# CCIG-Champalimaud/adell-mri

Measured on AMD Instinct MI355X. Metric: volumes/sec 3D U-Net 128^3 2-ch seg (train step: fwd+loss+bwd+SGD), higher is better.
Workload: dtype f32 (f16x3 split MFMA, fp32 accumulate); 1 GPU; BASELINE configs[1]: u-net-3d-resnet.yaml UNetPL, 2x128^3, batch 2/GPU, dice+focal, SGD-Nesterov; per_gpu_batch=2, parallelism=dp1, yaml=configs/u-net-3d-resnet.yaml, built_by=parse_config_unet -> get_segmentation_network('unet'), gradient_exchange=none (1 rank)

## Files before the change

adell_mri_amd/csrc/conv_fwd_s2.hip:

```cpp
#include <type_traits>
#include <utility>
#include "common.h"

typedef _Float16 half8 __attribute__((ext_vector_type(8)));
typedef _Float16 half4 __attribute__((ext_vector_type(4)));

namespace {

constexpr int kHX = 9, kHY = 9, kHZ = 5, kHV = kHX * kHY * kHZ;
constexpr int kWBytes = 27 * 2 * 32 * 64;
constexpr int kImg = kHV * 64;
constexpr int kCW = 4, kPW = 4;
constexpr int kThreads = (kCW + kPW) * 64, kPThreads = kPW * 64;
constexpr int kRedFloats = kCW * 32 * 2;
constexpr int kLds = kWBytes + 2 * kImg + 64 + kRedFloats * 4;
static_assert(kLds <= 160 * 1024, "one block per CU: weights + two half images");
constexpr int kItems = kHV * 4;
constexpr int kPer = (kItems + kPThreads - 1) / kPThreads;

template <typename T>
__device__ __forceinline__ ADELL_GLOBAL T* uniform_ptr(T* p) {
  const uint64_t v = reinterpret_cast<uint64_t>(p);
  const uint32_t lo = __builtin_amdgcn_readfirstlane((uint32_t)v);
  const uint32_t hi = __builtin_amdgcn_readfirstlane((uint32_t)(v >> 32));
  return reinterpret_cast<ADELL_GLOBAL T*>(((uint64_t)hi << 32) | lo);
}

template <int N, typename F, int... I>
__device__ __forceinline__ void static_for_impl(F&& body, std::integer_sequence<int, I...>) {
  (body(std::integral_constant<int, I>{}), ...);
}
template <int N, typename F>
__device__ __forceinline__ void static_for(F&& body) {
  static_for_impl<N>(body, std::make_integer_sequence<int, N>{});
}

struct FwdS2Args {
  const float* x;
  const char* wpack;
  const float* wscale;
  const float* bias;
  float* y;
  float* part;
  unsigned* amax_out;
  int N, D, H, W, Do, Ho, Wo;
  int ntx, nty, ntz;
  int nbricks;
};

}

#define ADELL_S2_BARRIER() asm volatile("s_waitcnt lgkmcnt(0)\n\ts_barrier" ::: "memory")

__device__ __forceinline__ int fwd_s2_scale_exp(float mx) {
  int kA = 0;
  const int ebits = (__float_as_int(mx) >> 23) & 0xff;
  if (ebits > 0 && ebits < 255) kA = 8 * ((13 - (ebits - 127)) >> 3);
  if (kA > 96) kA = 96;
  if (kA < -96) kA = -96;
  return kA;
}

__device__ __forceinline__ float fwd_s2_wave_max(float v) {
  auto step = [&](auto CTRL, auto ROWS) {
    const int o = __builtin_amdgcn_update_dpp(__float_as_int(v), __float_as_int(v), decltype(CTRL)::value,
                                              decltype(ROWS)::value, 0xf, false);
    v = fmaxf(v, __int_as_float(o));
  };
  step(std::integral_constant<int, 0xB1>{}, std::integral_constant<int, 0xf>{});
  step(std::integral_constant<int, 0x4E>{}, std::integral_constant<int, 0xf>{});
  step(std::integral_constant<int, 0x141>{}, std::integral_constant<int, 0xf>{});
  step(std::integral_constant<int, 0x140>{}, std::integral_constant<int, 0xf>{});
  step(std::integral_constant<int, 0x142>{}, std::integral_constant<int, 0xa>{});
  step(std::integral_constant<int, 0x143>{}, std::integral_constant<int, 0xc>{});
  return __int_as_float(__builtin_amdgcn_readlane(__float_as_int(v), 63));
}

template <int DBG>
__global__ __launch_bounds__(kThreads, 1) void adell_fwd_s2_fused_kernel(FwdS2Args a) {
  extern __shared__ char smem[];
  char* sW = smem;
  char* sA = smem + kWBytes;
  float* sMax = reinterpret_cast<float*>(sA + 2 * kImg);
  float* sRed = sMax + 16;
  const int tid = threadIdx.x, lane = tid & 63, wave = tid >> 6;
  const int li = lane & 31, lh = lane >> 5;
  const int nsp = a.ntx * a.nty * a.ntz;

  int first, stride, count;
  if (gridDim.x >= 8) {
    const int xcd = blockIdx.x & 7, per = (a.nbricks + 7) >> 3;
    const int lo = xcd * per, hi = (lo + per < a.nbricks) ? lo + per : a.nbricks;
    stride = gridDim.x >> 3;
    first = lo + (blockIdx.x >> 3);
    count = first < hi ? (hi - 1 - first) / stride + 1 : 0;
  } else {
    stride = gridDim.x;
    first = blockIdx.x;
    count = first < a.nbricks ? (a.nbricks - 1 - first) / stride + 1 : 0;
  }
  if (count == 0) return;
  const int nphases = count * 8;

  auto brick_origin = [&](int t, int& nb, int& tile, int& ox0, int& oy0, int& oz0) {
    tile = t % nsp;
    nb = t / nsp;
    int r = tile;
    const int tx = r % a.ntx;
    r /= a.ntx;
    const int ty = r % a.nty;
    const int tz = r / a.nty;
    ox0 = tx * 8;
    oy0 = ty * 8;
    oz0 = tz * 4;
  };

#pragma unroll 7
  for (int it = tid; it < 27 * 256; it += kThreads) {
    const float4 v = *reinterpret_cast<const float4*>(a.wpack + (size_t)it * 16);
    const int slot = it & 3, row = it >> 2;
    const int ch = row & 1, n = (row >> 1) & 31, tap = row >> 6;
    *reinterpret_cast<float4*>(sW + ((tap * 2 + ch) * 32 + n) * 64 + ((slot ^ ((n >> 2) & 3)) << 4)) = v;
  }

  if (wave >= kCW) {
    const int ptid = tid - kCW * 64, pw = wave - kCW;
    unsigned reloff[kPer], ldsoff[kPer];
#pragma unroll
    for (int u = 0; u < kPer; ++u) {
      int j = ptid + kPThreads * u;
      j = j < kItems ? j : j - kItems;
      const int hv = j >> 2, q4 = j & 3;
      const int hz = hv / (kHX * kHY), rem = hv - hz * (kHX * kHY);
      const int hy = rem / kHX, hx = rem - hy * kHX;
      reloff[u] = (unsigned)((2 * hz * a.H + 2 * hy) * a.W + 2 * hx) * 32u + 4u * q4;
      const int sw = (hv >> 2) & 3;
      ldsoff[u] = (unsigned)(hv * 64 + (q4 & 1) * 8 + (((q4 >> 1) ^ sw) << 4)) |
                  (unsigned)((hx << 16) | (hy << 20) | (hz << 24));
    }
    float4 raw[2][2][kPer];
    unsigned okbuf[2] = {0u, 0u};
    int pf_nb = 0, pf_ox0 = 0, pf_oy0 = 0, pf_oz0 = 0;
    auto issue = [&](int p, float4 (&f)[2][kPer], unsigned& okbits) {
      const int cls = p & 7;
      if (cls == 0) {
        int tile;
        brick_origin(first + (p >> 3) * stride, pf_nb, tile, pf_ox0, pf_oy0, pf_oz0);
        pf_nb = __builtin_amdgcn_readfirstlane(pf_nb);
        pf_ox0 = __builtin_amdgcn_readfirstlane(pf_ox0);
        pf_oy0 = __builtin_amdgcn_readfirstlane(pf_oy0);
        pf_oz0 = __builtin_amdgcn_readfirstlane(pf_oz0);
      }
      const int pz = cls >> 2, py = (cls >> 1) & 1, px = cls & 1;
      const int bz = 2 * (pf_oz0 - 1) + pz, by = 2 * (pf_oy0 - 1) + py, bx = 2 * (pf_ox0 - 1) + px;
      const ADELL_GLOBAL float* src = uniform_ptr(a.x + (size_t)pf_nb * a.D * a.H * a.W * 32);
      const bool inside = (bz >= 0) & (by >= 0) & (bx >= 0) & (bz + 2 * (kHZ - 1) < a.D) &
                          (by + 2 * (kHY - 1) < a.H) & (bx + 2 * (kHX - 1) < a.W);
      unsigned rel[kPer];
      unsigned ok = 0;
      if (inside) {
        const unsigned base = (unsigned)((bz * a.H + by) * a.W + bx) * 32u;
#pragma unroll
        for (int u = 0; u < kPer; ++u) rel[u] = base + reloff[u];
        ok = 0x80000000u;
      } else {
        const int base = ((bz * a.H + by) * a.W + bx) * 32;
#pragma unroll
        for (int u = 0; u < kPer; ++u) {
          const int hx = (ldsoff[u] >> 16) & 15, hy = (ldsoff[u] >> 20) & 15, hz = ldsoff[u] >> 24;
          const int iz = bz + 2 * hz, iy = by + 2 * hy, ix = bx + 2 * hx;
          const bool v = (iz >= 0) & (iz < a.D) & (iy >= 0) & (iy < a.H) & (ix >= 0) & (ix < a.W);
          rel[u] = v ? (unsigned)(base + (int)reloff[u]) : 0u;
          ok |= v ? (1u << u) : 0u;
        }
      }
      okbits = ok;
#pragma unroll
      for (int u = 0; u < kPer; ++u) {
        const f32x4 v0 = *reinterpret_cast<const ADELL_GLOBAL f32x4*>(src + rel[u]);
        const f32x4 v1 = *reinterpret_cast<const ADELL_GLOBAL f32x4*>(src + rel[u] + 16);
        f[0][u] = make_float4(v0.x, v0.y, v0.z, v0.w);
        f[1][u] = make_float4(v1.x, v1.y, v1.z, v1.w);
      }
    };
    auto publish_max = [&](float4 (&f)[2][kPer], unsigned okbits, int row) {
      float mx = 0.f;
#pragma unroll
      for (int c = 0; c < 2; ++c) {
        if (!(okbits >> 31)) {
#pragma unroll
          for (int u = 0; u < kPer; ++u) {
            const bool ok = (okbits >> u) & 1u;
            f[c][u] = make_float4(ok ? f[c][u].x : 0.f, ok ? f[c][u].y : 0.f, ok ? f[c][u].z : 0.f,
                                  ok ? f[c][u].w : 0.f);
          }
        }
#pragma unroll
        for (int u = 0; u < kPer; ++u)
          mx = fmaxf(fmaxf(fmaxf(mx, fabsf(f[c][u].x)), fmaxf(fabsf(f[c][u].y), fabsf(f[c][u].z))),
                     fabsf(f[c][u].w));
      }
      mx = fwd_s2_wave_max(mx);
      if (lane == 0) sMax[row * kPW + pw] = mx;
    };
    auto convert = [&](const float4 (&f)[kPer], float scaleA, char* img) {
#pragma unroll
      for (int u = 0; u < kPer; ++u) {
        if (!(DBG & 8)) {
          const float v[4] = {f[u].x * scaleA, f[u].y * scaleA, f[u].z * scaleA, f[u].w * scaleA};
          half4 h, l;
#pragma unroll
          for (int j = 0; j < 4; ++j) {
            h[j] = (_Float16)v[j];
            l[j] = (_Float16)(v[j] - (float)h[j]);
          }
          const unsigned off = ldsoff[u] & 0xffffu;
          *reinterpret_cast<half4*>(img + off) = h;
          *reinterpret_cast<half4*>(img + (off ^ 32u)) = l;
        }
      }
    };

    float block_max = 0.f;
    issue(0, raw[0], okbuf[0]);
    issue(1, raw[1], okbuf[1]);
    publish_max(raw[0], okbuf[0], 0);
    ADELL_S2_BARRIER();
    auto pstep = [&](int p, auto BUF) __attribute__((always_inline)) {
      constexpr int B = decltype(BUF)::value;
      const float* sm = sMax + kPW * (p & 1);
      const float mx = fmaxf(fmaxf(sm[0], sm[1]), fmaxf(sm[2], sm[3]));
      block_max = fmaxf(block_max, mx);
      const float scaleA = __int_as_float((fwd_s2_scale_exp(mx) + 127) << 23);
      const int pn = p + 2 < nphases ? p + 2 : nphases - 1;
      convert(raw[B][0], scaleA, sA);
      ADELL_S2_BARRIER();
      convert(raw[B][1], scaleA, sA + kImg);
      if (!((DBG & 16) && p > 1)) issue(pn, raw[B], okbuf[B]);
      publish_max(raw[1 - B], okbuf[1 - B], (p + 1) & 1);
      ADELL_S2_BARRIER();
    };
    for (int p = 0; p < nphases; p += 2) {
      pstep(p, std::integral_constant<int, 0>{});
      pstep(p + 1, std::integral_constant<int, 1>{});
    }
    ADELL_S2_BARRIER();
    if (a.amax_out != nullptr && ptid == 0) atomicMax(a.amax_out, __float_as_uint(block_max));
    return;
  }

  const int wz = wave;
  int arow[2];
#pragma unroll
  for (int mt = 0; mt < 2; ++mt) arow[mt] = (wz * kHY + (li >> 3) + 4 * mt) * kHX + (li & 7);
  const int bsw = (li >> 2) & 3;
  const int boffh = li * 64 + ((lh ^ bsw) << 4), boffl = li * 64 + (((2 + lh) ^ bsw) << 4);
  const float wsc = a.wscale[li];
  const float bcol = a.bias ? a.bias[li] : 0.f;
  f32x16 acc[2];
  int kprev = 0;

  auto taps = [&](int cls, auto CHT) __attribute__((always_inline)) {
    constexpr int ch = decltype(CHT)::value;
    const char* sAc = sA + ch * kImg;
    static_for<8>([&](auto CLS) {
      constexpr int c = decltype(CLS)::value;
      if (cls == c) {
        constexpr int pz = c >> 2, py = (c >> 1) & 1, px = c & 1;
        static_for<8>([&](auto T) {
          constexpr int tb = decltype(T)::value;
          constexpr int sz = tb >> 2, sy = (tb >> 1) & 1, sx = tb & 1;
          if constexpr ((sz <= pz) && (sy <= py) && (sx <= px) && !(DBG & 1)) {
            constexpr int tz = pz ? 2 * sz : 1, ty = py ? 2 * sy : 1, tx = px ? 2 * sx : 1;
            constexpr int dz = pz ? sz : 1, dy = py ? sy : 1, dx = px ? sx : 1;
            constexpr int tap = (tz * 3 + ty) * 3 + tx;
            const char* bt = sW + (tap * 2 + ch) * (32 * 64);
            const half8 bh = *reinterpret_cast<const half8*>(bt + boffh);
            const half8 bl = *reinterpret_cast<const half8*>(bt + boffl);
#pragma unroll
            for (int mt = 0; mt < 2; ++mt) {
              const int hv = arow[mt] + (dz * kHY + dy) * kHX + dx;
              const int sw = (hv >> 2) & 3;
              const char* row = sAc + hv * 64;
              const half8 ah = *reinterpret_cast<const half8*>(row + ((lh ^ sw) << 4));
              const half8 al = *reinterpret_cast<const half8*>(row + (((2 + lh) ^ sw) << 4));
              acc[mt] = __builtin_amdgcn_mfma_f32_32x32x16_f16(al, bh, acc[mt], 0, 0, 0);
              acc[mt] = __builtin_amdgcn_mfma_f32_32x32x16_f16(ah, bl, acc[mt], 0, 0, 0);
              acc[mt] = __builtin_amdgcn_mfma_f32_32x32x16_f16(ah, bh, acc[mt], 0, 0, 0);
            }
          }
        });
      }
    });
  };
  auto fold_stats = [&](int i) {
    if (a.part && tid < 32 && !(DBG & 2)) {
      int nb, tile, ox0, oy0, oz0;
      brick_origin(first + i * stride, nb, tile, ox0, oy0, oz0);
      float t1 = 0.f, t2 = 0.f;
#pragma unroll
      for (int w = 0; w < kCW; ++w) {
        t1 += sRed[(w * 32 + tid) * 2 + 0];
        t2 += sRed[(w * 32 + tid) * 2 + 1];
      }
      float* p = a.part + (((size_t)nb * nsp + tile) * 32 + tid) * 2;
      p[0] = t1;
      p[1] = t2;
    }
  };

  ADELL_S2_BARRIER();
  for (int p = 0; p < nphases; ++p) {
    const int cls = p & 7;
    {
      const float* sm = sMax + kPW * (p & 1);
      const float mx = fmaxf(fmaxf(sm[0], sm[1]), fmaxf(sm[2], sm[3]));
      const int kA = fwd_s2_scale_exp(mx);
      if (cls == 0) {
#pragma unroll
        for (int mt = 0; mt < 2; ++mt)
#pragma unroll
          for (int r = 0; r < 16; ++r) acc[mt][r] = 0.f;
      } else if (kA != kprev) {
        const float fix = __int_as_float((kA - kprev + 127) << 23);
#pragma unroll
        for (int mt = 0; mt < 2; ++mt)
#pragma unroll
          for (int r = 0; r < 16; ++r) acc[mt][r] *= fix;
      }
      kprev = kA;
    }
    ADELL_S2_BARRIER();
    if (cls == 0 && p > 0) fold_stats((p >> 3) - 1);
    taps(cls, std::integral_constant<int, 0>{});
    ADELL_S2_BARRIER();
    taps(cls, std::integral_constant<int, 1>{});
    if (cls == 7) {
      int nb, tile, ox0, oy0, oz0;
      brick_origin(first + (p >> 3) * stride, nb, tile, ox0, oy0, oz0);
      const float oscale = __int_as_float((127 - kprev) << 23) * wsc;
      const int z = oz0 + wz;
      float s1 = 0.f, s2 = 0.f;
      if (z < a.Do && !(DBG & 2)) {
#pragma unroll
        for (int mt = 0; mt < 2; ++mt)
#pragma unroll
          for (int r = 0; r < 16; ++r) {
            const int x = ox0 + (r & 3) + 4 * lh, yy = oy0 + (r >> 2) + 4 * mt;
            if (x < a.Wo && yy < a.Ho) {
              const float v = acc[mt][r] * oscale + bcol;
              a.y[((((size_t)nb * a.Do + z) * a.Ho + yy) * a.Wo + x) * 32 + li] = v;
              s1 += v;
              s2 += v * v;
            }
          }
      }
      if (a.part) {
        s1 += __shfl_xor(s1, 32, 64);
        s2 += __shfl_xor(s2, 32, 64);
        if (lh == 0) {
          sRed[(wz * 32 + li) * 2 + 0] = s1;
          sRed[(wz * 32 + li) * 2 + 1] = s2;
        }
      }
    }
  }
  ADELL_S2_BARRIER();
  if (count > 0) fold_stats(count - 1);
}

namespace {

bool fwd_s2_fused_ok(const adell_conv3d_desc* d) {
  return d && d->C1 == 0 && d->C0 == 32 && d->Cout == 32 && d->KD == 3 && d->KH == 3 && d->KW == 3 &&
         d->SD == 2 && d->SH == 2 && d->SW == 2 && d->PD == 1 && d->PH == 1 && d->PW == 1 &&
         d->D % 2 == 0 && d->H % 2 == 0 && d->W % 2 == 0 && d->N > 0 && d->D > 0 && d->H > 0 &&
         d->W > 0 && d->Do == d->D / 2 && d->Ho == d->H / 2 && d->Wo == d->W / 2 &&
         (size_t)d->D * d->H * d->W * 32 < ((size_t)1 << 29);
}

}

extern "C" int adell_conv3d_fwd_s2_fused_applicable(const adell_conv3d_desc* d) {
  return fwd_s2_fused_ok(d) ? 1 : 0;
}

extern "C" int adell_conv3d_fwd_s2_fused_ntiles(const adell_conv3d_desc* d) {
  if (!fwd_s2_fused_ok(d)) return ADELL_E_UNSUPPORTED;
  return adell_cdiv(d->Wo, 8) * adell_cdiv(d->Ho, 8) * adell_cdiv(d->Do, 4);
}

extern "C" int adell_conv3d_fwd_s2_fused(const adell_conv3d_desc* d, const float* x,
                                         const void* w_split, const float* wscale,
                                         const float* bias, float* y, float* stat_partials,
                                         int partial_rows, uint32_t* in_absmax, void* stream) {
  ADELL_REQUIRE(fwd_s2_fused_ok(d),
                "conv_fwd_s2_fused: needs 32 -> 32 channels, k = 3, stride 2, padding 1, even dims");
  ADELL_REQUIRE_ROWS(stat_partials, partial_rows,
                     (long)adell_cdiv(d->Wo, 8) * adell_cdiv(d->Ho, 8) * adell_cdiv(d->Do, 4),
                     "conv_fwd_s2_fused");
  ADELL_REQUIRE(x && w_split && wscale && y, "conv_fwd_s2_fused: null pointer");
  ADELL_REQUIRE(((uintptr_t)x & 15) == 0, "conv_fwd_s2_fused: x must be 16-byte aligned");
  FwdS2Args a;
  a.x = x;
  a.wpack = reinterpret_cast<const char*>(w_split);
  a.wscale = wscale;
  a.bias = bias;
  a.y = y;
  a.part = stat_partials;
  a.amax_out = in_absmax;
  a.N = d->N; a.D = d->D; a.H = d->H; a.W = d->W; a.Do = d->Do; a.Ho = d->Ho; a.Wo = d->Wo;
  a.ntx = adell_cdiv(d->Wo, 8);
  a.nty = adell_cdiv(d->Ho, 8);
  a.ntz = adell_cdiv(d->Do, 4);
  const long nbricks = (long)d->N * a.ntx * a.nty * a.ntz;
  ADELL_REQUIRE(nbricks < 0x0fffffffL, "conv_fwd_s2_fused: too many bricks");
  a.nbricks = (int)nbricks;
  int grid = (int)(nbricks < adell_cu_count() ? nbricks : adell_cu_count());
  if (grid >= 8) grid &= ~7;
  hipStream_t st = (hipStream_t)stream;
#ifdef ADELL_DEBUG
  switch (g_adell_tune.igemm_dbg) {
    case 1: return adell_launch<adell_fwd_s2_fused_kernel<1>>(dim3(grid), dim3(kThreads), kLds, st, a);
    case 2: return adell_launch<adell_fwd_s2_fused_kernel<2>>(dim3(grid), dim3(kThreads), kLds, st, a);
    case 3: return adell_launch<adell_fwd_s2_fused_kernel<3>>(dim3(grid), dim3(kThreads), kLds, st, a);
    case 8: return adell_launch<adell_fwd_s2_fused_kernel<8>>(dim3(grid), dim3(kThreads), kLds, st, a);
    case 16: return adell_launch<adell_fwd_s2_fused_kernel<16>>(dim3(grid), dim3(kThreads), kLds, st, a);
    case 27: return adell_launch<adell_fwd_s2_fused_kernel<27>>(dim3(grid), dim3(kThreads), kLds, st, a);
  }
#endif
  return adell_launch<adell_fwd_s2_fused_kernel<0>>(dim3(grid), dim3(kThreads), kLds, st, a);
}
```

Measured before the change: 63.32 volumes/s.

## Merge x-parity phases and stream per-phase weight slices through double-buffered LDS

The stride-2 fused conv kernel now stages both x-parity sub-images per phase, loading a contiguous 17-wide x row instead of strided samples. This halves the phase count from 8 to 4 per brick and doubles the producer waves from 4 to 8. The full 27-tap weight block no longer stays resident in LDS; only the taps a phase needs are streamed into two slices, prefetched into registers during the previous half-phase. This frees LDS for the larger images and cuts barriers per brick, at the cost of repeated weight reads from global/L2 and more register pressure.

```diff
diff --git a/adell_mri_amd/csrc/conv_fwd_s2.hip b/adell_mri_amd/csrc/conv_fwd_s2.hip
--- a/adell_mri_amd/csrc/conv_fwd_s2.hip
+++ b/adell_mri_amd/csrc/conv_fwd_s2.hip
@@ -8,15 +8,19 @@
 namespace {
 
 constexpr int kHX = 9, kHY = 9, kHZ = 5, kHV = kHX * kHY * kHZ;
-constexpr int kWBytes = 27 * 2 * 32 * 64;
-constexpr int kImg = kHV * 64;
-constexpr int kCW = 4, kPW = 4;
-constexpr int kThreads = (kCW + kPW) * 64, kPThreads = kPW * 64;
+constexpr int kMX = 2 * kHX - 1;
+constexpr int kSub = kHV * 64;
+constexpr int kImg = 2 * kSub;
+constexpr int kWSlice = 12 * 32 * 64;
+constexpr int kCW = 4, kPW = 8;
+constexpr int kThreads = (kCW + kPW) * 64, kPThreads = kPW * 64, kCThreads = kCW * 64;
 constexpr int kRedFloats = kCW * 32 * 2;
-constexpr int kLds = kWBytes + 2 * kImg + 64 + kRedFloats * 4;
-static_assert(kLds <= 160 * 1024, "one block per CU: weights + two half images");
-constexpr int kItems = kHV * 4;
+constexpr int kLds = 2 * kImg + 2 * kWSlice + 2 * kPW * 4 + kRedFloats * 4;
+static_assert(kLds <= 160 * 1024, "one block per CU: two half images + two weight slices");
+constexpr int kItems = kHZ * kHY * kMX * 4;
 constexpr int kPer = (kItems + kPThreads - 1) / kPThreads;
+static_assert(kPer * kPThreads - kItems <= kItems, "padding items repeat the first ones");
+constexpr int kWPer = 12 * 128 / kCThreads;
 
 template <typename T>
 __device__ __forceinline__ ADELL_GLOBAL T* uniform_ptr(T* p) {
@@ -79,10 +83,10 @@
 template <int DBG>
 __global__ __launch_bounds__(kThreads, 1) void adell_fwd_s2_fused_kernel(FwdS2Args a) {
   extern __shared__ char smem[];
-  char* sW = smem;
-  char* sA = smem + kWBytes;
-  float* sMax = reinterpret_cast<float*>(sA + 2 * kImg);
-  float* sRed = sMax + 16;
+  char* sA = smem;
+  char* sW = smem + 2 * kImg;
+  float* sMax = reinterpret_cast<float*>(sW + 2 * kWSlice);
+  float* sRed = sMax + 2 * kPW;
   const int tid = threadIdx.x, lane = tid & 63, wave = tid >> 6;
   const int li = lane & 31, lh = lane >> 5;
   const int nsp = a.ntx * a.nty * a.ntz;
@@ -100,7 +104,7 @@
     count = first < a.nbricks ? (a.nbricks - 1 - first) / stride + 1 : 0;
   }
   if (count == 0) return;
-  const int nphases = count * 8;
+  const int nphases = count * 4;
 
   auto brick_origin = [&](int t, int& nb, int& tile, int& ox0, int& oy0, int& oz0) {
     tile = t % nsp;
@@ -115,13 +119,13 @@
     oz0 = tz * 4;
   };
 
-#pragma unroll 7
-  for (int it = tid; it < 27 * 256; it += kThreads) {
-    const float4 v = *reinterpret_cast<const float4*>(a.wpack + (size_t)it * 16);
-    const int slot = it & 3, row = it >> 2;
-    const int ch = row & 1, n = (row >> 1) & 31, tap = row >> 6;
-    *reinterpret_cast<float4*>(sW + ((tap * 2 + ch) * 32 + n) * 64 + ((slot ^ ((n >> 2) & 3)) << 4)) = v;
-  }
+  auto phase_max = [&](int p) {
+    const float* sm = sMax + kPW * (p & 1);
+    float mx = sm[0];
+#pragma unroll
+    for (int w = 1; w < kPW; ++w) mx = fmaxf(mx, sm[w]);
+    return mx;
+  };
 
   if (wave >= kCW) {
     const int ptid = tid - kCW * 64, pw = wave - kCW;
@@ -130,47 +134,54 @@
     for (int u = 0; u < kPer; ++u) {
       int j = ptid + kPThreads * u;
       j = j < kItems ? j : j - kItems;
-      const int hv = j >> 2, q4 = j & 3;
-      const int hz = hv / (kHX * kHY), rem = hv - hz * (kHX * kHY);
-      const int hy = rem / kHX, hx = rem - hy * kHX;
-      reloff[u] = (unsigned)((2 * hz * a.H + 2 * hy) * a.W + 2 * hx) * 32u + 4u * q4;
+      const int v = j >> 2, q4 = j & 3;
+      const int row = v / kMX, m = v - row * kMX;
+      const int hz = row / kHY, hy = row - hz * kHY;
+      const int hx = (m + 1) >> 1, par = (m & 1) ^ 1;
+      const int hv = (hz * kHY + hy) * kHX + hx;
+      reloff[u] = (unsigned)((2 * hz * a.H + 2 * hy) * a.W + m) * 32u + 4u * q4;
       const int sw = (hv >> 2) & 3;
-      ldsoff[u] = (unsigned)(hv * 64 + (q4 & 1) * 8 + (((q4 >> 1) ^ sw) << 4)) |
-                  (unsigned)((hx << 16) | (hy << 20) | (hz << 24));
+      ldsoff[u] = (unsigned)(par * kSub + hv * 64 + (q4 & 1) * 8 + (((q4 >> 1) ^ sw) << 4)) |
+                  (unsigned)((m << 16) | (hy << 21) | (hz << 25));
     }
     float4 raw[2][2][kPer];
     unsigned okbuf[2] = {0u, 0u};
     int pf_nb = 0, pf_ox0 = 0, pf_oy0 = 0, pf_oz0 = 0;
     auto issue = [&](int p, float4 (&f)[2][kPer], unsigned& okbits) {
-      const int cls = p & 7;
+      const int cls = p & 3;
       if (cls == 0) {
         int tile;
-        brick_origin(first + (p >> 3) * stride, pf_nb, tile, pf_ox0, pf_oy0, pf_oz0);
+        brick_origin(first + (p >> 2) * stride, pf_nb, tile, pf_ox0, pf_oy0, pf_oz0);
         pf_nb = __builtin_amdgcn_readfirstlane(pf_nb);
         pf_ox0 = __builtin_amdgcn_readfirstlane(pf_ox0);
         pf_oy0 = __builtin_amdgcn_readfirstlane(pf_oy0);
         pf_oz0 = __builtin_amdgcn_readfirstlane(pf_oz0);
       }
-      const int pz = cls >> 2, py = (cls >> 1) & 1, px = cls & 1;
-      const int bz = 2 * (pf_oz0 - 1) + pz, by = 2 * (pf_oy0 - 1) + py, bx = 2 * (pf_ox0 - 1) + px;
+      const int pz = cls >> 1, py = cls & 1;
+      const int bz = 2 * (pf_oz0 - 1) + pz, by = 2 * (pf_oy0 - 1) + py, bx = 2 * pf_ox0 - 1;
       const ADELL_GLOBAL float* src = uniform_ptr(a.x + (size_t)pf_nb * a.D * a.H * a.W * 32);
+      const int skipy = py ? 0 : 2 * a.W * 32, skipz = pz ? 0 : 2 * a.H * a.W * 32;
       const bool inside = (bz >= 0) & (by >= 0) & (bx >= 0) & (bz + 2 * (kHZ - 1) < a.D) &
-                          (by + 2 * (kHY - 1) < a.H) & (bx + 2 * (kHX - 1) < a.W);
+                          (by + 2 * (kHY - 1) < a.H) & (bx + (kMX - 1) < a.W);
       unsigned rel[kPer];
       unsigned ok = 0;
       if (inside) {
         const unsigned base = (unsigned)((bz * a.H + by) * a.W + bx) * 32u;
 #pragma unroll
-        for (int u = 0; u < kPer; ++u) rel[u] = base + reloff[u];
+        for (int u = 0; u < kPer; ++u) {
+          const int hy = (ldsoff[u] >> 21) & 15, hz = ldsoff[u] >> 25;
+          rel[u] = base + reloff[u] + (unsigned)(hy == 0 ? skipy : 0) + (unsigned)(hz == 0 ? skipz : 0);
+        }
         ok = 0x80000000u;
       } else {
         const int base = ((bz * a.H + by) * a.W + bx) * 32;
 #pragma unroll
         for (int u = 0; u < kPer; ++u) {
-          const int hx = (ldsoff[u] >> 16) & 15, hy = (ldsoff[u] >> 20) & 15, hz = ldsoff[u] >> 24;
-          const int iz = bz + 2 * hz, iy = by + 2 * hy, ix = bx + 2 * hx;
+          const int m = (ldsoff[u] >> 16) & 31, hy = (ldsoff[u] >> 21) & 15, hz = ldsoff[u] >> 25;
+          const int ey = (hy == 0 && !py) ? 1 : hy, ez = (hz == 0 && !pz) ? 1 : hz;
+          const int iz = bz + 2 * ez, iy = by + 2 * ey, ix = bx + m;
           const bool v = (iz >= 0) & (iz < a.D) & (iy >= 0) & (iy < a.H) & (ix >= 0) & (ix < a.W);
-          rel[u] = v ? (unsigned)(base + (int)reloff[u]) : 0u;
+          rel[u] = v ? (unsigned)(base + (int)reloff[u] + (hy == 0 ? skipy : 0) + (hz == 0 ? skipz : 0)) : 0u;
           ok |= v ? (1u << u) : 0u;
         }
       }
@@ -228,8 +239,7 @@
     ADELL_S2_BARRIER();
     auto pstep = [&](int p, auto BUF) __attribute__((always_inline)) {
       constexpr int B = decltype(BUF)::value;
-      const float* sm = sMax + kPW * (p & 1);
-      const float mx = fmaxf(fmaxf(sm[0], sm[1]), fmaxf(sm[2], sm[3]));
+      const float mx = phase_max(p);
       block_max = fmaxf(block_max, mx);
       const float scaleA = __int_as_float((fwd_s2_scale_exp(mx) + 127) << 23);
       const int pn = p + 2 < nphases ? p + 2 : nphases - 1;
@@ -260,37 +270,75 @@
   f32x16 acc[2];
   int kprev = 0;
 
-  auto taps = [&](int cls, auto CHT) __attribute__((always_inline)) {
-    constexpr int ch = decltype(CHT)::value;
-    const char* sAc = sA + ch * kImg;
-    static_for<8>([&](auto CLS) {
-      constexpr int c = decltype(CLS)::value;
-      if (cls == c) {
-        constexpr int pz = c >> 2, py = (c >> 1) & 1, px = c & 1;
-        static_for<8>([&](auto T) {
-          constexpr int tb = decltype(T)::value;
-          constexpr int sz = tb >> 2, sy = (tb >> 1) & 1, sx = tb & 1;
-          if constexpr ((sz <= pz) && (sy <= py) && (sx <= px) && !(DBG & 1)) {
-            constexpr int tz = pz ? 2 * sz : 1, ty = py ? 2 * sy : 1, tx = px ? 2 * sx : 1;
-            constexpr int dz = pz ? sz : 1, dy = py ? sy : 1, dx = px ? sx : 1;
-            constexpr int tap = (tz * 3 + ty) * 3 + tx;
-            const char* bt = sW + (tap * 2 + ch) * (32 * 64);
-            const half8 bh = *reinterpret_cast<const half8*>(bt + boffh);
-            const half8 bl = *reinterpret_cast<const half8*>(bt + boffl);
-#pragma unroll
-            for (int mt = 0; mt < 2; ++mt) {
-              const int hv = arow[mt] + (dz * kHY + dy) * kHX + dx;
-              const int sw = (hv >> 2) & 3;
-              const char* row = sAc + hv * 64;
-              const half8 ah = *reinterpret_cast<const half8*>(row + ((lh ^ sw) << 4));
-              const half8 al = *reinterpret_cast<const half8*>(row + (((2 + lh) ^ sw) << 4));
-              acc[mt] = __builtin_amdgcn_mfma_f32_32x32x16_f16(al, bh, acc[mt], 0, 0, 0);
-              acc[mt] = __builtin_amdgcn_mfma_f32_32x32x16_f16(ah, bl, acc[mt], 0, 0, 0);
-              acc[mt] = __builtin_amdgcn_mfma_f32_32x32x16_f16(ah, bh, acc[mt], 0, 0, 0);
-            }
+  const ADELL_GLOBAL char* wsrc = uniform_ptr(a.wpack);
+  auto slice_load = [&](auto KT, int ch, float4 (&wr)[kWPer]) __attribute__((always_inline)) {
+    constexpr int K = decltype(KT)::value, pz = K >> 1, py = K & 1;
+    constexpr int nit = 3 * (1 + pz) * (1 + py) * 128;
+    int tt = tid;
+    asm volatile("" : "+v"(tt));
+    static_for<kWPer>([&](auto U) {
+      constexpr int u = decltype(U)::value;
+      if constexpr (kCThreads * u < nit) {
+        int it = tt + kCThreads * u;
+        it = it < nit ? it : nit - 1;
+        const int slot = it & 3, n = (it >> 2) & 31, sidx = it >> 7;
+        const int g = sidx / 3, tx = sidx - 3 * g;
+        const int iz = py ? g >> 1 : g, iy = py ? g & 1 : 0;
+        const int tap = ((pz ? 2 * iz : 1) * 3 + (py ? 2 * iy : 1)) * 3 + tx;
+        const f32x4 v = *reinterpret_cast<const ADELL_GLOBAL f32x4*>(
+            wsrc + (unsigned)(((tap * 32 + n) * 2 + ch) * 64 + slot * 16));
+        wr[u] = make_float4(v.x, v.y, v.z, v.w);
+      }
+    });
+  };
+  auto slice_store = [&](auto KT, int ch, const float4 (&wr)[kWPer]) __attribute__((always_inline)) {
+    constexpr int K = decltype(KT)::value, pz = K >> 1, py = K & 1;
+    constexpr int nit = 3 * (1 + pz) * (1 + py) * 128;
+    int tt = tid;
+    asm volatile("" : "+v"(tt));
+    static_for<kWPer>([&](auto U) {
+      constexpr int u = decltype(U)::value;
+      if constexpr (kCThreads * u < nit) {
+        const int it = tt + kCThreads * u;
+        if (kCThreads * (u + 1) <= nit || it < nit) {
+          const int slot = it & 3, n = (it >> 2) & 31, sidx = it >> 7;
+          *reinterpret_cast<float4*>(sW + ch * kWSlice + (sidx * 32 + n) * 64 + ((slot ^ ((n >> 2) & 3)) << 4)) =
+              wr[u];
+        }
+      }
+    });
+  };
+
+  auto taps = [&](auto KT, auto CHT) __attribute__((always_inline)) {
+    constexpr int K = decltype(KT)::value, ch = decltype(CHT)::value;
+    constexpr int pz = K >> 1, py = K & 1;
+    int arow_b[2] = {arow[0], arow[1]};
+    asm volatile("" : "+v"(arow_b[0]), "+v"(arow_b[1]));
+    static_for<2>([&](auto PX) {
+      constexpr int px = decltype(PX)::value;
+      const char* sAc = sA + ch * kImg + px * kSub;
+      static_for<8>([&](auto T) {
+        constexpr int tb = decltype(T)::value;
+        constexpr int sz = tb >> 2, sy = (tb >> 1) & 1, sx = tb & 1;
+        if constexpr ((sz <= pz) && (sy <= py) && (sx <= px) && !(DBG & 1)) {
+          constexpr int dz = pz ? sz : 1, dy = py ? sy : 1, dx = px ? sx : 1;
+          constexpr int sidx = ((pz ? sz : 0) * (1 + py) + (py ? sy : 0)) * 3 + (px ? 2 * sx : 1);
+          const char* bt = sW + ch * kWSlice + sidx * (32 * 64);
+          const half8 bh = *reinterpret_cast<const half8*>(bt + boffh);
+          const half8 bl = *reinterpret_cast<const half8*>(bt + boffl);
+#pragma unroll
+          for (int mt = 0; mt < 2; ++mt) {
+            const int hv = arow_b[mt] + (dz * kHY + dy) * kHX + dx;
+            const int sw = (hv >> 2) & 3;
+            const char* row = sAc + hv * 64;
+            const half8 ah = *reinterpret_cast<const half8*>(row + ((lh ^ sw) << 4));
+            const half8 al = *reinterpret_cast<const half8*>(row + (((2 + lh) ^ sw) << 4));
+            acc[mt] = __builtin_amdgcn_mfma_f32_32x32x16_f16(al, bh, acc[mt], 0, 0, 0);
+            acc[mt] = __builtin_amdgcn_mfma_f32_32x32x16_f16(ah, bl, acc[mt], 0, 0, 0);
+            acc[mt] = __builtin_amdgcn_mfma_f32_32x32x16_f16(ah, bh, acc[mt], 0, 0, 0);
           }
-        });
-      }
+        }
+      });
     });
   };
   auto fold_stats = [&](int i) {
@@ -309,12 +357,26 @@
     }
   };
 
+  auto half_phase = [&](int p, auto KT, auto CHT) __attribute__((always_inline)) {
+    constexpr int K = decltype(KT)::value, ch = decltype(CHT)::value;
+    constexpr int NK = ch ? ((K + 1) & 3) : K, nch = 1 - ch;
+    float4 wr[kWPer];
+    slice_load(std::integral_constant<int, NK>{}, nch, wr);
+    ADELL_S2_BARRIER();
+    if (K == 0 && ch == 0 && p > 0) fold_stats((p >> 2) - 1);
+    taps(KT, CHT);
+    slice_store(std::integral_constant<int, NK>{}, nch, wr);
+  };
+  {
+    float4 wr[kWPer];
+    slice_load(std::integral_constant<int, 0>{}, 0, wr);
+    slice_store(std::integral_constant<int, 0>{}, 0, wr);
+  }
   ADELL_S2_BARRIER();
   for (int p = 0; p < nphases; ++p) {
-    const int cls = p & 7;
+    const int cls = p & 3;
     {
-      const float* sm = sMax + kPW * (p & 1);
-      const float mx = fmaxf(fmaxf(sm[0], sm[1]), fmaxf(sm[2], sm[3]));
+      const float mx = phase_max(p);
       const int kA = fwd_s2_scale_exp(mx);
       if (cls == 0) {
 #pragma unroll
@@ -330,14 +392,15 @@
       }
       kprev = kA;
     }
-    ADELL_S2_BARRIER();
-    if (cls == 0 && p > 0) fold_stats((p >> 3) - 1);
-    taps(cls, std::integral_constant<int, 0>{});
-    ADELL_S2_BARRIER();
-    taps(cls, std::integral_constant<int, 1>{});
-    if (cls == 7) {
+    static_for<4>([&](auto KT) {
+      if (cls == decltype(KT)::value) {
+        half_phase(p, KT, std::integral_constant<int, 0>{});
+        half_phase(p, KT, std::integral_constant<int, 1>{});
+      }
+    });
+    if (cls == 3) {
       int nb, tile, ox0, oy0, oz0;
-      brick_origin(first + (p >> 3) * stride, nb, tile, ox0, oy0, oz0);
+      brick_origin(first + (p >> 2) * stride, nb, tile, ox0, oy0, oz0);
       const float oscale = __int_as_float((127 - kprev) << 23) * wsc;
       const int z = oz0 + wz;
       float s1 = 0.f, s2 = 0.f;
```

Result: no change. 63.37 volumes/s (median of 4 runs) (+0.1%).
